# AIM-SE/AC-TSR

Hardware: AMD Instinct MI355X
Metric: user-sequences/sec fwd+bwd, AC-SASRec L=50 d=64, 1/2/4/8 MI355X (higher is better)
Workload: dtype f32; 1 GPU; ACSASRec full training step (spatial + adversarial calibrators, BASELINE configs[2]), synthetic 100000-item catalogue, B=512/GPU L=50 d=64 h=2 2 layers inner=256, CE loss, two-pass backward + Adam; global_batch=512, seq_len=50, hidden=64, heads=2, parallelism=dp1, launch=hipGraph replay per step, backward=two walks (reference protocol, trainer.py:672-686)

## Files before the change

### ac_tsr_amd/_lib.py

```python
from __future__ import annotations

import ctypes as C
import os
import subprocess

_HERE = os.path.dirname(os.path.abspath(__file__))
CSRC = os.path.join(_HERE, "csrc")
LIB_PATH = os.environ.get("ACATTN_LIB") or os.path.join(CSRC, "libacattn.so")
HEADER_PATH = os.path.join(os.path.dirname(_HERE), "include", "acattn.h")

ABI_VERSION = 34
MAX_MASKS = 8
NSTAT = 8
MASK_STRUCTURED, MASK_DENSE_LL, MASK_DENSE_L = 0, 1, 2
COMBINE = {"fixed": 0, "gate": 1, "annealing": 2}
RICH = {"none": 0, "fixed": 1, "trainable": 2}
RNG_EXPLICIT, RNG_COUNTER = 0, 1
FWD_AUTO, FWD_STREAM, FWD_STAGED, FWD_GENERAL, FWD_LONG = 0, 1, 2, 3, 4
BWD_AUTO, BWD_STREAM, BWD_ROW, BWD_LONG = 0, 1, 2, 3

_f = C.c_void_p


class Problem(C.Structure):
# ... 106 lines not shown

class EmbedProblem(C.Structure):
    _fields_ = [("rows", C.c_int32), ("L", C.c_int32), ("H", C.c_int32), ("n_table_rows", C.c_int64), ("idx", _f),
                ("table", _f), ("pos", _f), ("gamma", _f), ("beta", _f), ("eps", C.c_float), ("p_drop", C.c_float),
                ("keep", _f), ("seed", C.c_uint64), ("seed_device", _f), ("nonzero_out", _f), ("hot_id_plus1", C.c_int64)]


EMBED_BWD_CHUNKS = 8
PENALTY_WS_FLOATS = 1024
WGRAD_MAX_GROUP = 8
WGRAD_MAX_REDUCE = 32
SUMROWS_MAX_DEFER = 8

SYMBOLS = {
    "acattn_abi_version": (C.c_int, []),
    "acattn_max_sequence_length": (C.c_int, []),
    "acattn_calibrated_attention_bwd_gate_summed": (C.c_int, [C.POINTER(Problem), C.POINTER(BwdIO)]),
    "acattn_calibrated_attention_bwd_pair_supported": (C.c_int, [C.POINTER(Problem), C.POINTER(BwdIO)]),
    "acattn_last_error": (C.c_char_p, []),
    "acattn_fwd_algorithmic_bytes": (C.c_int64, [C.POINTER(Problem)]),
    "acattn_calibrated_attention_fwd": (C.c_int, [C.POINTER(Problem), C.POINTER(FwdOut), C.c_void_p]),
    "acattn_calibrated_attention_bwd": (C.c_int, [C.POINTER(Problem), C.POINTER(BwdIO), C.c_void_p]),
    "acattn_calibrated_attention_bwd_attack_side": (C.c_int, [C.POINTER(Problem), C.POINTER(BwdIO), C.c_void_p]),
    "acattn_spatial_attention_bwd": (C.c_int, [C.POINTER(Problem), C.POINTER(SpatialBwdIO), C.c_void_p]),
    "acattn_spatial_attention_bwd_workspace_bytes": (C.c_int64, [C.POINTER(Problem)]),
    "acattn_spatial_affines": (C.c_int, [C.POINTER(Problem), _f, C.c_void_p]),
    "acattn_full_sort_ce_workspace_bytes": (C.c_int64, [C.POINTER(CeProblem)]),
    "acattn_full_sort_ce_fwd": (C.c_int, [C.POINTER(CeProblem), _f, _f, _f, C.c_void_p]),
    "acattn_full_sort_ce_fwd_dir": (C.c_int, [C.POINTER(CeProblem), _f, _f, _f, _f, C.c_void_p]),
    "acattn_full_sort_ce_bwd": (C.c_int, [C.POINTER(CeProblem), _f, _f, _f, _f, _f, C.c_void_p]),
    "acattn_full_sort_ce_fwd_pair_workspace_bytes": (C.c_int64, [C.POINTER(CeProblem), C.POINTER(CeProblem)]),
    "acattn_full_sort_ce_fwd_pair": (C.c_int, [C.POINTER(CeProblem), C.POINTER(CeProblem), _f, _f, _f, _f, _f, _f, C.c_void_p]),
    "acattn_full_sort_ce_products": (C.c_int, [C.c_int]),
    "acattn_linear_products": (C.c_int, [C.c_int]),
    "acattn_dropout_add_layernorm_fwd": (C.c_int, [C.POINTER(LnProblem), _f, _f, C.c_void_p]),
    "acattn_dropout_add_layernorm_bwd": (C.c_int, [C.POINTER(LnProblem), _f, _f, _f, _f, _f, C.c_void_p]),
    "acattn_embed_layernorm_fwd": (C.c_int, [C.POINTER(EmbedProblem), _f, _f, C.c_void_p]),
    "acattn_embed_layernorm_bwd": (C.c_int, [C.POINTER(EmbedProblem), _f, _f, C.c_int64, _f, _f, _f, C.c_void_p]),
    "acattn_projections_supported": (C.c_int, [C.c_int32, C.c_int32]),
    "acattn_projections_bwd_workspace_bytes": (C.c_int64, [C.POINTER(ProjProblem)]),
    "acattn_projections_fwd": (C.c_int, [C.POINTER(ProjProblem), C.POINTER(ProjOut), C.c_void_p]),
    "acattn_projections_qkv_supported": (C.c_int, [C.c_int32]),
    "acattn_projections_qkv_fwd": (C.c_int, [C.POINTER(ProjProblem), C.POINTER(ProjOut), C.c_void_p]),
    "acattn_projections_bwd": (C.c_int, [C.POINTER(ProjProblem), C.POINTER(ProjBwdIO), C.c_void_p]),
    "acattn_layer_tail_supported": (C.c_int, [C.c_int32, C.c_int32]),
    "acattn_layer_tail_fwd": (C.c_int, [C.POINTER(TailProblem), C.POINTER(TailSaved), C.c_void_p]),
# ... 99 lines not shown
```

### ac_tsr_amd/csrc/acattn_api.hip

```cpp
#include <stdint.h>
#include <stdio.h>
#include <string.h>

#include <algorithm>

#include "acattn_common.h"

namespace {
thread_local char g_err[256] = "";
constexpr int ACATTN_MAX_L = 496;

int fail(const char* msg) {
  snprintf(g_err, sizeof(g_err), "%s", msg);
  return -1;
}

int check_problem(const acattn_problem* p) {
  if (!p) return fail("problem is NULL");
  if (p->B < 1 || p->L < 1 || p->H < 1 || p->n_heads < 1) return fail("B, L, H, n_heads must be positive");
  if (p->H % p->n_heads != 0)
    return fail("The hidden size is not a multiple of the number of attention heads");
  const int dh = p->H / p->n_heads;
  if (dh != 16 && dh != 32 && dh != 64 && dh != 128) return fail("unsupported head size: dh must be 16, 32, 64 or 128");
  if (p->L > ACATTN_MAX_L) return fail("unsupported sequence length: L must be <= 496 (acattn_max_sequence_length)");
// ... 15 lines not shown
    if (p->adversarial && !p->two_level && !p->keep_before) return fail("explicit dropout needs keep_before");
  }
  if (p->adversarial) {
    if (!p->qa || !p->ka) return fail("adversarial calibrator needs qa and ka");
    if (p->rng_mode == ACATTN_RNG_EXPLICIT && !p->noise) return fail("explicit rng mode needs noise");
    if (p->combine_option == ACATTN_COMBINE_GATE) {
      if (!p->gate_logits) return fail("combine_option gate needs gate_logits");
    } else if (p->combine_option != ACATTN_COMBINE_FIXED && p->combine_option != ACATTN_COMBINE_ANNEALING) {
      return fail("unknown combine_option");
    }
    if (!p->two_level) {
      if (p->rich_combine != ACATTN_RICH_FIXED && p->rich_combine != ACATTN_RICH_TRAINABLE)
        return fail("unknown rich_calibrated_combine");
      if (p->rich_combine == ACATTN_RICH_TRAINABLE && !p->rich_ratio) return fail("trainable rich combine needs rich_ratio");
    }
  }
  return 0;
}
}

void acattn_set_error(const char* msg) { snprintf(g_err, sizeof(g_err), "%s", msg); }

int acattn_launch_bwd_attack(const acattn_problem& p, const acattn_bwd_io& io, hipStream_t stream, float* gate_zero);

extern "C" {

int acattn_abi_version(void) { return ACATTN_ABI_VERSION; }

int acattn_max_sequence_length(void) { return ACATTN_MAX_L; }

int acattn_select_forward_kernel(int which) { return acattn_fwd_kernel_choice(which); }

int acattn_select_backward_kernel(int which) { return acattn_bwd_kernel_choice(which); }

const char* acattn_last_error(void) { return g_err; }

int64_t acattn_fwd_algorithmic_bytes(const acattn_problem* p) {
  if (!p) return -1;
  const int64_t t_lh = 4LL * p->L * p->H, t_ll = 4LL * p->L * p->L;
  if (!p->adversarial) return (int64_t)p->B * 4 * t_lh;
  int64_t per_seq = 7 * t_lh + (int64_t)p->n_heads * t_ll;
  if (p->combine_option == ACATTN_COMBINE_GATE) per_seq += t_ll;
  return (int64_t)p->B * per_seq;
}

int acattn_calibrated_attention_fwd(const acattn_problem* p, const acattn_fwd_out* out, void* stream) {
// ... 24 lines not shown
int acattn_calibrated_attention_bwd(const acattn_problem* p, const acattn_bwd_io* io, void* stream) {
  if (int rc = check_problem(p)) return rc;
  if (!io) return fail("io is NULL");
  if (!p->adversarial) return fail("backward is defined for the adversarial (full) operator only");
  if (!io->attack_mask || !io->row_stats) return fail("backward needs the forward's attack_mask and row_stats");
  if (!io->dq || !io->dk || !io->dv || !io->dqa || !io->dka) return fail("dq, dk, dv, dqa, dka must be non-NULL");
  if (p->combine_option == ACATTN_COMBINE_GATE && !io->dgate_logits) return fail("gate combine needs dgate_logits");
  if (!io->dw_order_part || !io->dw_dist_part || !io->dsmall_part) return fail("parameter partial buffers must be non-NULL");
  if (io->part_stride != 0 && io->part_stride < 2 * (p->H / p->n_heads)) return fail("part_stride is smaller than a partial row");
  const int rc = acattn_launch_bwd(*p, *io, (hipStream_t)stream);
  if (rc > 0) snprintf(g_err, sizeof(g_err), "HIP launch failed: %s", hipGetErrorString((hipError_t)rc));
  return rc;
}

int acattn_calibrated_attention_bwd_attack_side(const acattn_problem* p, const acattn_bwd_io* io, void* stream) {
  if (int rc = check_problem(p)) return rc;
  if (!io) return fail("io is NULL");
  if (!p->adversarial) return fail("backward is defined for the adversarial (full) operator only");
  if (!io->attack_mask || !io->row_stats) return fail("backward needs the forward's attack_mask and row_stats");
  if (!io->dqa || !io->dka) return fail("dqa, dka must be non-NULL");
  const int rc = acattn_launch_bwd_attack(*p, *io, (hipStream_t)stream, nullptr);
  if (rc > 0) snprintf(g_err, sizeof(g_err), "HIP launch failed: %s", hipGetErrorString((hipError_t)rc));
  if (rc == -100) snprintf(g_err, sizeof(g_err), "the attack-side backward (acattn_bwd_attack.hip) does not cover this launch");
  return rc;
}

int acattn_calibrated_attention_bwd_gate_summed(const acattn_problem* p, const acattn_bwd_io* io) {
  if (!p || !io || p->B < 1 || p->L < 1 || p->H < 1 || p->n_heads < 1) return 0;
  return acattn_bwd_gate_summed(*p, *io) ? 1 : 0;
}

int acattn_calibrated_attention_bwd_pair_supported(const acattn_problem* p, const acattn_bwd_io* io) {
  if (!p || !io || p->B < 1 || p->L < 1 || p->H < 1 || p->n_heads < 1) return 0;
  return acattn_bwd_pair_supported(*p, *io) ? 1 : 0;
}

int64_t acattn_calibrated_attention_bwd_workspace_bytes(const acattn_problem* p) {
  if (!p || p->B < 1 || p->L < 1 || p->n_heads < 1) return -1;
  const bool long_form = p->L > 208 || acattn_bwd_kernel_choice(-1) == ACATTN_BWD_LONG;
  return (long_form ? 2 : 1) * acattn_bwd_stream_ws_bytes(*p);
}

int acattn_spatial_attention_bwd(const acattn_problem* p, const acattn_spatial_bwd_io* io, void* stream) {
  if (int rc = check_problem(p)) return rc;
  if (!io) return fail("io is NULL");
  if (p->L > 208) return fail("the spatial-only backward is built for sequence length L <= 208 (the long form covers the forward and acattn_calibrated_attention_bwd)");
// ... 592 lines not shown
```

### ac_tsr_amd/csrc/acattn_bwd.hip

```cpp
#include <stdlib.h>

#include "acattn_common.h"

int acattn_launch_bwd_general_dh16(const acattn_problem& p, const acattn_bwd_io& io, hipStream_t stream);
int acattn_launch_bwd_general_dh32(const acattn_problem& p, const acattn_bwd_io& io, hipStream_t stream);
int acattn_launch_bwd_general_dh64(const acattn_problem& p, const acattn_bwd_io& io, hipStream_t stream);
int acattn_launch_bwd_general_dh128(const acattn_problem& p, const acattn_bwd_io& io, hipStream_t stream);

int acattn_launch_bwd_fast(const acattn_problem& p, const acattn_bwd_io& io, hipStream_t stream);
int acattn_launch_bwd_stream(const acattn_problem& p, const acattn_bwd_io& io, hipStream_t stream);
int acattn_launch_bwd_attack(const acattn_problem& p, const acattn_bwd_io& io, hipStream_t stream, float* gate_zero = nullptr);
int acattn_launch_bwd_onerow(const acattn_problem& p, const acattn_bwd_io& io, bool accumulate, hipStream_t stream, bool gate_zeroed = false);
int acattn_launch_bwd_long(const acattn_problem& p, const acattn_bwd_io& io, hipStream_t stream);

namespace {
thread_local int g_bwd_kernel = ACATTN_BWD_AUTO;
}
int acattn_bwd_kernel_choice(int which) {
  const int old = g_bwd_kernel;
  if (which >= ACATTN_BWD_AUTO && which <= ACATTN_BWD_LONG) g_bwd_kernel = which;
  return old;
}

bool acattn_bwd_onerow_applies(const acattn_problem& p, const acattn_bwd_io& io);

namespace {
bool attack_kernel_enabled() {
  static const bool on = getenv("ACATTN_BWD_ATTACK") ? atoi(getenv("ACATTN_BWD_ATTACK")) != 0 : true;
  return on;
}
bool onerow_split_applies(const acattn_problem& p, const acattn_bwd_io& io) {
  static const bool split = getenv("ACATTN_ONEROW_SPLIT") ? atoi(getenv("ACATTN_ONEROW_SPLIT")) != 0 : true;
  if (!(split && (io.d_attack_mask || io.d_penalty_part) && io.read_rows && io.n_read_rows == 1 && !io.active_qblocks && !io.attack_only && p.L <= 64))
    return false;
// ... 51 lines not shown
      if (rc_mask == 0) {
        acattn_bwd_io row_io = io;
        row_io.d_attack_mask = nullptr;
        row_io.d_penalty_part = nullptr;
        const int rc_row = acattn_launch_bwd_onerow(p, row_io, true, stream, gate_zeroed);
        if (rc_row != -100) return rc_row;
        acattn_set_error("attention backward: the mask-only launch ran but the one-row kernel does not cover this problem (read-row chain not computed)");
        return -1;
      }
      if (rc_mask != -100) return rc_mask;
    }
    if (io.dgate_summed) {
      acattn_set_error("attention backward: dgate_summed was accepted but no one-row form ran");
      return -1;
    }
  }
  static const bool short_stream = getenv("ACATTN_BWD_SHORT_STREAM") && atoi(getenv("ACATTN_BWD_SHORT_STREAM")) != 0;
  const bool short_rows = p.L <= 64 && !short_stream;
  if (which == ACATTN_BWD_AUTO && short_rows) {
    if (io.attack_only && attack_kernel_enabled()) {
      const int rc_attack = acattn_launch_bwd_attack(p, io, stream);
      if (rc_attack != -100) return rc_attack;
    }
    const int rc_fast = acattn_launch_bwd_fast(p, io, stream);
    if (rc_fast != -100) return rc_fast;
  }
  if (which == ACATTN_BWD_AUTO || which == ACATTN_BWD_STREAM) {
    const int rc_stream = acattn_launch_bwd_stream(p, io, stream);
    if (rc_stream != -100) return rc_stream;
  }
  const int rc_fast = acattn_launch_bwd_fast(p, io, stream);
  if (rc_fast != -100) return rc_fast;
  switch (p.H / p.n_heads) {
    case 16: return acattn_launch_bwd_general_dh16(p, io, stream);
    case 32: return acattn_launch_bwd_general_dh32(p, io, stream);
    case 64: return acattn_launch_bwd_general_dh64(p, io, stream);
    case 128: return acattn_launch_bwd_general_dh128(p, io, stream);
  }
  return -1;
}
```

### ac_tsr_amd/csrc/acattn_bwd_attack.hip

```cpp
#include <stdlib.h>

#include <type_traits>

#include "acattn_common.h"

namespace {

constexpr float kLog2e = 1.44269504088896340736f;
constexpr float kLn2 = 0.69314718055994530942f;

__device__ __forceinline__ float ex2(float x) { return __builtin_amdgcn_exp2f(x); }
__device__ __forceinline__ float hsum(const f4 v) { return (v[0] + v[1]) + (v[2] + v[3]); }

constexpr int TS = 20;

__device__ __forceinline__ int again(int x) {
  asm volatile("" : "+v"(x));
  return x;
}

__device__ __forceinline__ void rng_keep_pair(const RngKey key, uint32_t row_id, uint32_t grp, float p_drop, uint32_t& keep_after,
                                              uint32_t& keep_mask) {
  if (p_drop == 0.5f) {
    uint32_t x = (row_id * 64u + grp) ^ key.a;
    x *= 0x7feb352dU;
    x ^= x >> 15;
    x *= 0x846ca68bU;
    x ^= x >> 16;
    x += key.b;
    const uint32_t w2 = rng_word(x, 0xB5297A4Du, 0x85EBCA77u);
    keep_after = (w2 >> 4) & 0xFu;
    keep_mask = (w2 >> 12) & 0xFu;
  } else {
    const RngGroup rg = rng_group(key, row_id, grp, p_drop);
    keep_after = rg.keep_after;
    keep_mask = rg.keep_mask;
  }
}

template <int DH, bool CTX>
__global__ void __launch_bounds__(256, CTX ? 3 : 4) acattn_bwd_attack_kernel(const acattn_problem P, const acattn_bwd_io IO, float* gate_zero,
                                                                    const int n_slots) {
  constexpr int KS = DH / 4;
  constexpr int DT = DH / 16;
  constexpr int VS = DH + 4;
  constexpr int SLOT = 16 * VS;

  const int L = P.L, H = P.H, nh = P.n_heads;
  const int nT = (L + 15) >> 4;
  const int LP = nT * 16;
  int b, h;
  decode_block(blockIdx.x, P.B, nh, b, h);
  const int lane = threadIdx.x & 63;
  const int wave = __builtin_amdgcn_readfirstlane(threadIdx.x >> 6);
  const int c = lane & 15, g = lane >> 4;
  const size_t rowbase = (size_t)b * L;
  const int hoff = h * DH;
  const size_t bh = (size_t)b * nh + h;

  extern __shared__ __attribute__((aligned(16))) float smem[];
// ... 486 lines not shown
```

### ac_tsr_amd/csrc/acattn_common.h

```cpp
#pragma once
#include <hip/hip_runtime.h>
#include <stdint.h>

#include <type_traits>

#include "acattn.h"

typedef float f4 __attribute__((ext_vector_type(4)));
typedef float f4u __attribute__((ext_vector_type(4), aligned(4)));

#define ACATTN_NEG_INF (-__builtin_inff())
#define ACATTN_MASK_FILL (-10000.0f)
#define ACATTN_LOG_EPS (1e-24f)

__device__ __forceinline__ float quad_sum(float x) {
  auto r = __builtin_amdgcn_permlane16_swap(__float_as_uint(x), __float_as_uint(x), false, false);
  x = __uint_as_float(r[0]) + __uint_as_float(r[1]);
  auto s = __builtin_amdgcn_permlane32_swap(__float_as_uint(x), __float_as_uint(x), false, false);
  return __uint_as_float(s[0]) + __uint_as_float(s[1]);
}

__device__ __forceinline__ float quad_max(float x) {
  auto r = __builtin_amdgcn_permlane16_swap(__float_as_uint(x), __float_as_uint(x), false, false);
  x = fmaxf(__uint_as_float(r[0]), __uint_as_float(r[1]));
// ... 157 lines not shown
    const float u2 = (float)(wn[pair] & 0xFFFFu) * (1.0f / 65536.0f);
    const float rad = __builtin_amdgcn_sqrtf(__builtin_amdgcn_logf(u1) * (-2.0f * 0.69314718055994530942f)) * scale;
    acattn_f2 cs = {__builtin_amdgcn_cosf(u2), __builtin_amdgcn_sinf(u2)};
    asm("" : "+v"(cs));
    n[pair] = cs * rad;
  }
  o.n01 = n[0];
  o.n23 = n[1];
  const uint32_t w2 = rng_word(x, 0xB5297A4Du, 0x85EBCA77u);
  o.keep_after = (w2 >> 4) & 0xFu;
  o.keep_mask = (w2 >> 12) & 0xFu;
  o.keep_before = (w2 >> 20) & 0xFu;
  return o;
}

__device__ __forceinline__ uint32_t rng_keep_mask_half(const RngKey key, uint32_t row_id, uint32_t grp) {
  uint32_t x = (row_id * 64u + grp) ^ key.a;
  x *= 0x7feb352dU;
  x ^= x >> 15;
  x *= 0x846ca68bU;
  x ^= x >> 16;
  x += key.b;
  return (rng_word(x, 0xB5297A4Du, 0x85EBCA77u) >> 12) & 0xFu;
}

__device__ __forceinline__ f4 keep_scale4(uint32_t bits, float keep_scale) {
  f4 s;
#pragma unroll
  for (int r = 0; r < 4; ++r) s[r] = ((bits >> r) & 1u) ? keep_scale : 0.f;
  return s;
}
__device__ __forceinline__ int sbit(uint32_t bits, int idx) {
  int m = __builtin_amdgcn_sbfe(bits, idx, 1);
  asm("" : "+v"(m));
  return m;
}
__device__ __forceinline__ float keep_and(float x, uint32_t bits, int r) {
  return __uint_as_float(__float_as_uint(x) & (uint32_t)sbit(bits, r));
}

__device__ __forceinline__ void store_out4(float* p, const f4 v) { __builtin_nontemporal_store(v, (f4*)p); }
__device__ __forceinline__ void store_out1(float* p, const float v) { __builtin_nontemporal_store(v, p); }

__device__ __forceinline__ bool qblock_has_ctx(const acattn_bwd_io& IO, int b, int qb) {
  if (IO.active_qblocks) return (IO.active_qblocks[b] >> qb) & 1u;
  if (IO.read_rows) {
// ... 130 lines not shown
```

### include/acattn.h

```cpp
#ifndef ACATTN_H_
#define ACATTN_H_

#include <stdint.h>

#ifdef __cplusplus
extern "C" {
#endif

#define ACATTN_ABI_VERSION 34

enum {
  ACATTN_MASK_STRUCTURED = 0,
  ACATTN_MASK_DENSE_LL = 1,
  ACATTN_MASK_DENSE_L = 2
};

enum { ACATTN_COMBINE_FIXED = 0, ACATTN_COMBINE_GATE = 1, ACATTN_COMBINE_ANNEALING = 2 };

enum { ACATTN_RICH_NONE = 0, ACATTN_RICH_FIXED = 1, ACATTN_RICH_TRAINABLE = 2 };

enum {
  ACATTN_RNG_EXPLICIT = 0,
  ACATTN_RNG_COUNTER = 1
};
// ... 369 lines not shown
                           uint8_t* keep_after, uint8_t* keep_mask, uint8_t* keep_before, void* stream);

enum {
  ACATTN_FWD_AUTO = 0,
  ACATTN_FWD_STREAM = 1,
  ACATTN_FWD_STAGED = 2,
  ACATTN_FWD_GENERAL = 3,
  ACATTN_FWD_LONG = 4
};
int acattn_select_forward_kernel(int which);

int acattn_max_sequence_length(void);

enum {
  ACATTN_BWD_AUTO = 0,
  ACATTN_BWD_STREAM = 1,
  ACATTN_BWD_ROW = 2,
  ACATTN_BWD_LONG = 3
};
int acattn_select_backward_kernel(int which);

int acattn_calibrated_attention_bwd_attack_side(const acattn_problem* p, const acattn_bwd_io* io, void* stream);

#ifdef __cplusplus
}
#endif
#endif
```

Measured before the change: 540,500 user-sequences/sec.

## Add specialised calibrated-walk attention backward kernel for short sequences

Adds a new fused backward kernel for the calibrated (non-attack) walk of the two-pass backward. It is dispatched ahead of the generic fast backward when L<=64, the mask is structured, gate combine and two-level are set, and RNG is counter-based. The kernel keeps K, Ka and V in LDS, computes the spatial and score gradients per 16-row query block with MFMA, and reduces the key-side gradients through LDS slots, either all at once or in turns when LDS is short. The aim is to replace the general kernel with one that avoids redundant traffic and launches for this shape, at the cost of a large new code path and high LDS use that may limit occupancy.

Result: no change. 545,600 user-sequences/sec, median of 6 (+0.9%).

```diff
diff --git a/ac_tsr_amd/_lib.py b/ac_tsr_amd/_lib.py
--- a/ac_tsr_amd/_lib.py
+++ b/ac_tsr_amd/_lib.py
@@ -152,6 +152,7 @@
     "acattn_calibrated_attention_fwd": (C.c_int, [C.POINTER(Problem), C.POINTER(FwdOut), C.c_void_p]),
     "acattn_calibrated_attention_bwd": (C.c_int, [C.POINTER(Problem), C.POINTER(BwdIO), C.c_void_p]),
     "acattn_calibrated_attention_bwd_attack_side": (C.c_int, [C.POINTER(Problem), C.POINTER(BwdIO), C.c_void_p]),
+    "acattn_calibrated_attention_bwd_cal": (C.c_int, [C.POINTER(Problem), C.POINTER(BwdIO), C.c_void_p]),
     "acattn_spatial_attention_bwd": (C.c_int, [C.POINTER(Problem), C.POINTER(SpatialBwdIO), C.c_void_p]),
     "acattn_spatial_attention_bwd_workspace_bytes": (C.c_int64, [C.POINTER(Problem)]),
     "acattn_spatial_affines": (C.c_int, [C.POINTER(Problem), _f, C.c_void_p]),
diff --git a/ac_tsr_amd/csrc/acattn_api.hip b/ac_tsr_amd/csrc/acattn_api.hip
--- a/ac_tsr_amd/csrc/acattn_api.hip
+++ b/ac_tsr_amd/csrc/acattn_api.hip
@@ -61,6 +61,7 @@
 void acattn_set_error(const char* msg) { snprintf(g_err, sizeof(g_err), "%s", msg); }
 
 int acattn_launch_bwd_attack(const acattn_problem& p, const acattn_bwd_io& io, hipStream_t stream, float* gate_zero);
+int acattn_launch_bwd_cal(const acattn_problem& p, const acattn_bwd_io& io, hipStream_t stream);
 
 extern "C" {
 
@@ -131,6 +132,19 @@
   const int rc = acattn_launch_bwd_attack(*p, *io, (hipStream_t)stream, nullptr);
   if (rc > 0) snprintf(g_err, sizeof(g_err), "HIP launch failed: %s", hipGetErrorString((hipError_t)rc));
   if (rc == -100) snprintf(g_err, sizeof(g_err), "the attack-side backward (acattn_bwd_attack.hip) does not cover this launch");
+  return rc;
+}
+
+int acattn_calibrated_attention_bwd_cal(const acattn_problem* p, const acattn_bwd_io* io, void* stream) {
+  if (int rc = check_problem(p)) return rc;
+  if (!io) return fail("io is NULL");
+  if (!p->adversarial) return fail("backward is defined for the adversarial (full) operator only");
+  if (!io->attack_mask || !io->row_stats) return fail("backward needs the forward's attack_mask and row_stats");
+  if (!io->dq || !io->dk || !io->dv || !io->dqa || !io->dka) return fail("dq, dk, dv, dqa, dka must be non-NULL");
+  if (io->part_stride != 0 && io->part_stride < 2 * (p->H / p->n_heads)) return fail("part_stride is smaller than a partial row");
+  const int rc = acattn_launch_bwd_cal(*p, *io, (hipStream_t)stream);
+  if (rc > 0) snprintf(g_err, sizeof(g_err), "HIP launch failed: %s", hipGetErrorString((hipError_t)rc));
+  if (rc == -100) snprintf(g_err, sizeof(g_err), "the calibrated-walk backward (acattn_bwd_cal.hip) does not cover this launch");
   return rc;
 }
 
diff --git a/ac_tsr_amd/csrc/acattn_bwd.hip b/ac_tsr_amd/csrc/acattn_bwd.hip
--- a/ac_tsr_amd/csrc/acattn_bwd.hip
+++ b/ac_tsr_amd/csrc/acattn_bwd.hip
@@ -10,6 +10,7 @@
 int acattn_launch_bwd_fast(const acattn_problem& p, const acattn_bwd_io& io, hipStream_t stream);
 int acattn_launch_bwd_stream(const acattn_problem& p, const acattn_bwd_io& io, hipStream_t stream);
 int acattn_launch_bwd_attack(const acattn_problem& p, const acattn_bwd_io& io, hipStream_t stream, float* gate_zero = nullptr);
+int acattn_launch_bwd_cal(const acattn_problem& p, const acattn_bwd_io& io, hipStream_t stream);
 int acattn_launch_bwd_onerow(const acattn_problem& p, const acattn_bwd_io& io, bool accumulate, hipStream_t stream, bool gate_zeroed = false);
 int acattn_launch_bwd_long(const acattn_problem& p, const acattn_bwd_io& io, hipStream_t stream);
 
@@ -107,6 +108,10 @@
       const int rc_attack = acattn_launch_bwd_attack(p, io, stream);
       if (rc_attack != -100) return rc_attack;
     }
+    if (!io.attack_only) {
+      const int rc_cal = acattn_launch_bwd_cal(p, io, stream);
+      if (rc_cal != -100) return rc_cal;
+    }
     const int rc_fast = acattn_launch_bwd_fast(p, io, stream);
     if (rc_fast != -100) return rc_fast;
   }
diff --git a/ac_tsr_amd/csrc/acattn_bwd_attack.hip b/ac_tsr_amd/csrc/acattn_bwd_attack.hip
--- a/ac_tsr_amd/csrc/acattn_bwd_attack.hip
+++ b/ac_tsr_amd/csrc/acattn_bwd_attack.hip
@@ -17,25 +17,6 @@
 __device__ __forceinline__ int again(int x) {
   asm volatile("" : "+v"(x));
   return x;
-}
-
-__device__ __forceinline__ void rng_keep_pair(const RngKey key, uint32_t row_id, uint32_t grp, float p_drop, uint32_t& keep_after,
-                                              uint32_t& keep_mask) {
-  if (p_drop == 0.5f) {
-    uint32_t x = (row_id * 64u + grp) ^ key.a;
-    x *= 0x7feb352dU;
-    x ^= x >> 15;
-    x *= 0x846ca68bU;
-    x ^= x >> 16;
-    x += key.b;
-    const uint32_t w2 = rng_word(x, 0xB5297A4Du, 0x85EBCA77u);
-    keep_after = (w2 >> 4) & 0xFu;
-    keep_mask = (w2 >> 12) & 0xFu;
-  } else {
-    const RngGroup rg = rng_group(key, row_id, grp, p_drop);
-    keep_after = rg.keep_after;
-    keep_mask = rg.keep_mask;
-  }
 }
 
 template <int DH, bool CTX>
diff --git a/ac_tsr_amd/csrc/acattn_bwd_cal.hip b/ac_tsr_amd/csrc/acattn_bwd_cal.hip
--- /dev/null
+++ b/ac_tsr_amd/csrc/acattn_bwd_cal.hip
@@ -0,0 +1,686 @@
+#include <stdlib.h>
+
+#include <type_traits>
+
+#include "acattn_common.h"
+
+namespace {
+
+constexpr float kLog2e = 1.44269504088896340736f;
+
+__device__ __forceinline__ float ex2(float x) { return __builtin_amdgcn_exp2f(x); }
+__device__ __forceinline__ float hsum(const f4 v) { return (v[0] + v[1]) + (v[2] + v[3]); }
+
+__device__ __forceinline__ float row16_sum(float v) {
+  v += __builtin_bit_cast(float, __builtin_amdgcn_update_dpp(0, __builtin_bit_cast(int, v), 0xB1, 0xF, 0xF, false));
+  v += __builtin_bit_cast(float, __builtin_amdgcn_update_dpp(0, __builtin_bit_cast(int, v), 0x4E, 0xF, 0xF, false));
+  v += __builtin_bit_cast(float, __builtin_amdgcn_update_dpp(0, __builtin_bit_cast(int, v), 0x141, 0xF, 0xF, false));
+  v += __builtin_bit_cast(float, __builtin_amdgcn_update_dpp(0, __builtin_bit_cast(int, v), 0x140, 0xF, 0xF, false));
+  return v;
+}
+
+__device__ __forceinline__ uint32_t again(uint32_t x) {
+  asm volatile("" : "+v"(x));
+  return x;
+}
+
+constexpr int TS = 20;
+
+#ifdef ACATTN_BWD_STAMPS
+__device__ unsigned long long g_bwd_cal_stamps[8192 * 16];
+#define BWD_STAMP(k)                                                                  \
+  do {                                                                                \
+    __builtin_amdgcn_sched_barrier(0);                                                \
+    asm volatile("s_memtime %0\n\ts_waitcnt lgkmcnt(0)" : "=s"(stamp_[k])::"memory"); \
+    __builtin_amdgcn_sched_barrier(0);                                                \
+  } while (0)
+#else
+#define BWD_STAMP(k)
+#endif
+
+template <int DH>
+__global__ void __launch_bounds__(256, 2) acattn_bwd_cal_kernel(const acattn_problem P, const acattn_bwd_io IO, const int n_slots) {
+  constexpr int KS = DH / 4;
+  constexpr int DT = DH / 16;
+  constexpr int VS = DH + 4;
+  constexpr int SLOT = 16 * VS;
+  constexpr int CP = 2 * DH + 4;
+
+  const int L = P.L, H = P.H, nh = P.n_heads;
+  const int nT = (L + 15) >> 4;
+  const int LP = nT * 16;
+  int b, h;
+  decode_block(blockIdx.x, P.B, nh, b, h);
+  const int lane = threadIdx.x & 63;
+  const int wave = __builtin_amdgcn_readfirstlane(threadIdx.x >> 6);
+  const int c = lane & 15, g = lane >> 4;
+  const size_t rowbase = (size_t)b * L;
+  const int hoff = h * DH;
+  const size_t bh = (size_t)b * nh + h;
+#ifdef ACATTN_BWD_STAMPS
+  unsigned long long stamp_[16] = {};
+#endif
+  BWD_STAMP(0);
+
+  extern __shared__ __attribute__((aligned(16))) float smem[];
+  float* Ks = smem;
+  float* Kas = Ks + LP * VS;
+  float* Vs = Kas + LP * VS;
+  float* slots_k = smem;
+  float* slots_ka = slots_k + n_slots * SLOT;
+  float* slots_v = smem + max(3 * LP * VS, 2 * n_slots * SLOT);
+  float* s_co = slots_v + n_slots * SLOT;
+  float* s_cd = s_co + LP;
+  float* s_km = s_cd + LP;
+  float* s_lt = s_km + LP;
+  float* s_kh = s_lt + LP;
+  float* scr_all = s_kh + nT * 2 * DH;
+  float* part_all = scr_all + nT * 16 * TS;
+  float* scr = scr_all + wave * 16 * TS;
+  float* my_part = part_all + wave * (2 * LP + CP);
+  const int PW = 2 * LP + CP;
+
+  const int qb = wave;
+  const int i0 = qb * 16, i = i0 + c;
+  const bool row_ok = i < L;
+  float qf[KS], qaf[KS];
+  {
+    const size_t off = (rowbase + (row_ok ? i : 0)) * H + hoff + KS * g;
+#pragma unroll
+    for (int s4 = 0; s4 < KS / 4; ++s4) {
+      f4 t = {0.f, 0.f, 0.f, 0.f}, ta = t;
+      if (row_ok) {
+        t = *(const f4*)(P.q + off + 4 * s4);
+        ta = *(const f4*)(P.qa + off + 4 * s4);
+      }
+#pragma unroll
+      for (int e = 0; e < 4; ++e) {
+        qf[4 * s4 + e] = t[e];
+        qaf[4 * s4 + e] = ta[e];
+      }
+    }
+  }
+  float lse_x2 = 0.f, lse_y2 = 0.f, lse_v2 = 0.f, lse_w2 = 0.f;
+  if (row_ok) {
+    const float* sp = IO.row_stats + (bh * L + i) * ACATTN_NSTAT;
+    lse_x2 = sp[0] * kLog2e;
+    lse_y2 = sp[1] * kLog2e;
+    lse_v2 = sp[3] * kLog2e;
+    lse_w2 = sp[4] * kLog2e;
+  }
+
+  constexpr int KV_IT = DH / 16;
+  f4 r_k[KV_IT], r_ka[KV_IT], r_v[KV_IT];
+#pragma unroll
+  for (int it = 0; it < KV_IT; ++it) {
+    const int idx = threadIdx.x + it * blockDim.x;
+    const int row = idx / (DH / 4), c4 = idx - row * (DH / 4);
+    r_k[it] = f4{0.f, 0.f, 0.f, 0.f};
+    r_ka[it] = r_k[it];
+    r_v[it] = r_k[it];
+    if (row < L) {
+      const size_t o = (rowbase + row) * H + hoff + 4 * c4;
+      r_k[it] = *(const f4*)(P.k + o);
+      r_ka[it] = *(const f4*)(P.ka + o);
+      r_v[it] = *(const f4*)(P.v + o);
+    }
+  }
+  const f4 w_ko = *(const f4*)(P.w_order + DH + 4 * (threadIdx.x % (DH / 4)));
+  const f4 w_kd = *(const f4*)(P.w_dist + DH + 4 * (threadIdx.x % (DH / 4)));
+  const uint8_t r_valid = (threadIdx.x < L) ? P.key_valid[rowbase + threadIdx.x] : (uint8_t)0;
+  BWD_STAMP(1);
+#pragma unroll
+  for (int it = 0; it < KV_IT; ++it) {
+    const int idx = threadIdx.x + it * blockDim.x;
+    const int row = idx / (DH / 4), c4 = idx - row * (DH / 4);
+    const f4 kv = r_k[it];
+    *(f4*)(Ks + row * VS + 4 * c4) = kv;
+    *(f4*)(Kas + row * VS + 4 * c4) = r_ka[it];
+    *(f4*)(Vs + row * VS + 4 * c4) = r_v[it];
+    float co = kv.x * w_ko.x + kv.y * w_ko.y + kv.z * w_ko.z + kv.w * w_ko.w;
+    float cd = kv.x * w_kd.x + kv.y * w_kd.y + kv.z * w_kd.z + kv.w * w_kd.w;
+#pragma unroll
+    for (int off = 1; off < DH / 4; off <<= 1) {
+      co += __shfl_xor(co, off);
+      cd += __shfl_xor(cd, off);
+    }
+    if (c4 == 0) {
+      s_co[row] = -kLog2e * co;
+      s_cd[row] = cd;
+    }
+  }
+  if (threadIdx.x < LP) {
+    const int j = threadIdx.x;
+    float km = ACATTN_NEG_INF;
+    if (j < L) km = r_valid ? 0.f : ACATTN_MASK_FILL * kLog2e;
+    s_km[j] = km;
+    s_lt[j] = logf((float)(j + 1));
+  }
+
+  float ao = 0.f, ad = 0.f;
+#pragma unroll
+  for (int s4 = 0; s4 < KS / 4; ++s4) {
+    const f4 a = *(const f4*)(P.w_order + KS * g + 4 * s4), d = *(const f4*)(P.w_dist + KS * g + 4 * s4);
+#pragma unroll
+    for (int e = 0; e < 4; ++e) {
+      ao += qf[4 * s4 + e] * a[e];
+      ad += qf[4 * s4 + e] * d[e];
+    }
+  }
+  ao = quad_sum(ao) + P.b_order[0];
+  ad = quad_sum(ad) + P.b_dist[0];
+  const float sc = P.scalar[0];
+  const uint64_t seed_eff = P.seed + (P.seed_device ? *P.seed_device : 0ull);
+  const RngKey rkey = rng_key(seed_eff);
+  __syncthreads();
+  BWD_STAMP(2);
+
+  const unsigned long long valid_keys = __ballot(lane < L && s_km[lane] == 0.f);
+  const int first_valid = valid_keys ? __ffsll((long long)valid_keys) - 1 : L;
+  const bool causal = P.causal != 0;
+  const int nt_valid = valid_keys ? ((63 - __clzll((long long)valid_keys)) >> 4) + 1 : nT;
+  auto tiles_of_block = [&](int q) {
+    const bool rows_see_a_key = causal ? first_valid <= 16 * q : valid_keys != 0;
+    return rows_see_a_key ? min(causal ? min(nT, q + 1) : nT, nt_valid) : nT;
+  };
+  int nts[4], base[4], total = 0;
+#pragma unroll
+  for (int q = 0; q < 4; ++q) {
+    nts[q] = q < nT ? tiles_of_block(q) : 0;
+    base[q] = total;
+    total += nts[q];
+  }
+  const int nt = tiles_of_block(qb);
+  const int my_base = qb == 0 ? base[0] : qb == 1 ? base[1] : qb == 2 ? base[2] : base[3];
+  const bool in_turns = total > n_slots;
+
+  const float s2 = sc * sc;
+  const float inv_sqrt = 1.0f / sqrtf((float)DH);
+  const float scale2 = inv_sqrt * kLog2e;
+  const float ao2 = -kLog2e * ao;
+  const float nc2 = -(0.5f * s2 * scale2);
+  const bool has_drop = P.p_drop > 0.f;
+  const float keep_scale = has_drop ? 1.0f / (1.0f - P.p_drop) : 1.0f;
+  const uint32_t prow = ((uint32_t)bh * L + (row_ok ? i : 0)) * (uint32_t)L;
+  const uint32_t rng_row = (uint32_t)(bh * L + i);
+  const float okf = row_ok ? 1.0f : 0.0f;
+
+  auto mask4 = [&](int t) -> f4 {
+    const f4 km4 = *(const f4*)(s_km + 16 * t + 4 * g);
+    if (causal && (16 * t + 15 > i0)) {
+      const int dq = (c - 4 * g) + 16 * (qb - t);
+      f4 m;
+#pragma unroll
+      for (int r = 0; r < 4; ++r) m[r] = (dq < r) ? fminf(km4[r], ACATTN_MASK_FILL * kLog2e) : km4[r];
+      return m;
+    }
+    return km4;
+  };
+  auto spatial = [&](int t, f4& pr, f4& val, f4& df) {
+    const f4 ea = *(const f4*)(s_co + 16 * t + 4 * g) + ao2;
+    const f4 cd4 = *(const f4*)(s_cd + 16 * t + 4 * g);
+    const int d0 = i - (16 * t + 4 * g);
+    f4 lt4;
+    if (16 * t + 15 > i0) {
+#pragma unroll
+      for (int r = 0; r < 4; ++r) {
+        pr[r] = fast_rcp(1.0f + ex2(ea[r]));
+        val[r] = (d0 - r < 0) ? pr[r] : 1.0f - pr[r];
+        lt4[r] = s_lt[d0 - r < 0 ? r - d0 : d0 - r];
+      }
+    } else {
+      const float* lp = s_lt + d0;
+#pragma unroll
+      for (int r = 0; r < 4; ++r) {
+        pr[r] = fast_rcp(1.0f + ex2(ea[r]));
+        val[r] = 1.0f - pr[r];
+        lt4[r] = lp[-r];
+      }
+    }
+    df = lt4 - (cd4 + ad);
+  };
+  auto load_seg = [&](const float* base, int t) -> f4 {
+    const int j0 = 16 * t + 4 * g;
+    f4 v = {0.f, 0.f, 0.f, 0.f};
+    if (row_ok && j0 < L) {
+      const float* p = base + j0;
+      if (j0 + 3 < L) {
+        v = *(const f4u*)p;
+      } else {
+#pragma unroll
+        for (int r = 0; r < 4; ++r)
+          if (j0 + r < L) v[r] = p[r];
+      }
+    }
+    return v;
+  };
+  auto store_seg = [&](float* base, int t, const f4 val) {
+    const int j0 = 16 * t + 4 * g;
+    if (!row_ok || j0 >= L) return;
+    float* p = base + j0;
+    if (j0 + 3 < L) {
+      *(f4u*)p = val;
+    } else {
+#pragma unroll
+      for (int r = 0; r < 4; ++r)
+        if (j0 + r < L) p[r] = val[r];
+    }
+  };
+  auto load_cols = [&](const float* src, float (&col)[4][DT]) {
+#pragma unroll
+    for (int s = 0; s < 4; ++s) {
+      const int row = i0 + 4 * g + s;
+      const float* p = src + (rowbase + min(row, L - 1)) * H + hoff + c;
+#pragma unroll
+      for (int dt = 0; dt < DT; ++dt) col[s][dt] = row < L ? p[16 * dt] : 0.f;
+    }
+  };
+
+  auto body = [&](auto ntb_c) {
+    constexpr int NTB = decltype(ntb_c)::value;
+    asm volatile("; %0 key tiles" ::"n"(NTB) : "memory");
+
+    auto score_tiles = [&](const float* Xs, const float (&frag)[KS], f4 (&out)[NTB]) {
+#pragma unroll
+      for (int t = 0; t < NTB; ++t) out[t] = f4{0.f, 0.f, 0.f, 0.f};
+#pragma unroll
+      for (int s4 = 0; s4 < KS / 4; ++s4) {
+#pragma unroll
+        for (int t = 0; t < NTB; ++t) {
+          const f4 x4 = *(const f4*)(Xs + (16 * t + c) * VS + KS * g + 4 * s4);
+#pragma unroll
+          for (int e = 0; e < 4; ++e) out[t] = mfma16(x4[e], frag[4 * s4 + e], out[t]);
+        }
+      }
+    };
+    auto key_side = [&](const f4 (&tile)[NTB], const float (&col)[4][DT], auto sink) {
+#pragma unroll
+      for (int t = 0; t < NTB; ++t) {
+        asm volatile("s_waitcnt lgkmcnt(0)" ::: "memory");
+        *(f4*)(scr + c * TS + 4 * g) = tile[t];
+        asm volatile("s_waitcnt lgkmcnt(0)" ::: "memory");
+        f4 o[DT];
+#pragma unroll
+        for (int dt = 0; dt < DT; ++dt) o[dt] = f4{0.f, 0.f, 0.f, 0.f};
+#pragma unroll
+        for (int s = 0; s < 4; ++s) {
+          const float b_t = scr[(4 * g + s) * TS + c];
+#pragma unroll
+          for (int dt = 0; dt < DT; ++dt) o[dt] = mfma16(col[s][dt], b_t, o[dt]);
+        }
+        sink(t, o);
+      }
+    };
+    auto park = [&](const f4 (&tile)[NTB], const float (&col)[4][DT], float* area) {
+      if (!in_turns) {
+        key_side(tile, col, [&](int t, const f4 (&o)[DT]) {
+          float* sl = area + (my_base + t) * SLOT + c * VS + 4 * g;
+#pragma unroll
+          for (int dt = 0; dt < DT; ++dt) *(f4*)(sl + 16 * dt) = o[dt];
+        });
+      } else {
+        for (int j = lane; j < SLOT; j += 64) area[wave * SLOT + j] = 0.f;
+        __syncthreads();
+        for (int q = 0; q < nT; ++q) {
+          if (q == qb)
+            key_side(tile, col, [&](int t, const f4 (&o)[DT]) {
+              float* sl = area + t * SLOT + c * VS + 4 * g;
+#pragma unroll
+              for (int dt = 0; dt < DT; ++dt) *(f4*)(sl + 16 * dt) += o[dt];
+            });
+          __syncthreads();
+        }
+      }
+    };
+
+    constexpr bool EARLY = DH <= 32;
+    f4 gc[KS / 4];
+    float gcc[4][DT];
+    auto load_gc = [&] {
+      const size_t off = (rowbase + (row_ok ? i : 0)) * H + hoff + KS * g;
+#pragma unroll
+      for (int s4 = 0; s4 < KS / 4; ++s4) {
+        gc[s4] = f4{0.f, 0.f, 0.f, 0.f};
+        if (row_ok) gc[s4] = *(const f4*)(IO.d_ctx_calibrated + off + 4 * s4);
+      }
+    };
+    if constexpr (EARLY) {
+      load_gc();
+      load_cols(IO.d_ctx_calibrated, gcc);
+    }
+
+    f4 tS[NTB], tM[NTB];
+    score_tiles(Ks, qf, tS);
+    score_tiles(Kas, qaf, tM);
+#pragma unroll
+    for (int t = 0; t < NTB; ++t) {
+      const f4 mk4 = mask4(t);
+      f4 pr, val, df;
+      spatial(t, pr, val, df);
+      f4 lg;
+#pragma unroll
+      for (int r = 0; r < 4; ++r) lg[r] = __builtin_amdgcn_logf(val[r] + ACATTN_LOG_EPS);
+      f4 x = tS[t] * scale2 + mk4;
+      x = lg * inv_sqrt + x;
+      x = (df * df) * nc2 + x;
+#pragma unroll
+      for (int r = 0; r < 4; ++r) tS[t][r] = ex2(x[r] - lse_x2) * okf;
+      const f4 y = tM[t] * scale2 + mk4;
+#pragma unroll
+      for (int r = 0; r < 4; ++r) tM[t][r] = ex2(y[r] - lse_y2) * okf;
+    }
+    BWD_STAMP(3);
+
+    uint32_t keepA = 0, keepM = 0;
+#pragma unroll
+    for (int t = 0; t < NTB; ++t) {
+      uint32_t ka = 0xFu, km = 0xFu;
+      if (has_drop) rng_keep_pair(rkey, rng_row, (uint32_t)(4 * t + g), P.p_drop, ka, km);
+      keepA |= ka << (4 * t);
+      keepM |= km << (4 * t);
+    }
+    BWD_STAMP(4);
+
+    f4 dPa[NTB], dMa[NTB];
+    {
+      f4 dAw[NTB], Ac[NTB], Aw[NTB];
+#pragma unroll
+      for (int t = 0; t < NTB; ++t) dAw[t] = f4{0.f, 0.f, 0.f, 0.f};
+      if constexpr (!EARLY) load_gc();
+#pragma unroll
+      for (int s4 = 0; s4 < KS / 4; ++s4) {
+#pragma unroll
+        for (int t = 0; t < NTB; ++t) {
+          const f4 x4 = *(const f4*)(Vs + (16 * t + c) * VS + KS * g + 4 * s4);
+#pragma unroll
+          for (int e = 0; e < 4; ++e) dAw[t] = mfma16(x4[e], gc[s4][e], dAw[t]);
+        }
+      }
+      const float* grow = P.gate_logits + (rowbase + (row_ok ? i : 0)) * L;
+      float dc = 0.f;
+#pragma unroll
+      for (int t = 0; t < NTB; ++t) {
+        const f4 sa = keep_scale4((keepA >> (4 * t)) & 0xFu, keep_scale), sm = keep_scale4((keepM >> (4 * t)) & 0xFu, keep_scale);
+        const f4 p = tS[t] * sa, m = tM[t] * sm;
+        const f4 mk4 = mask4(t);
+        const f4 a1 = m * (-kLog2e) + kLog2e;
+        f4 ex1;
+#pragma unroll
+        for (int r = 0; r < 4; ++r) ex1[r] = ex2(a1[r]);
+        const f4 v2 = (p * ex1) * kLog2e + (mk4 - lse_v2);
+        const f4 gt = gate_value(load_seg(grow, t), P.gate_is_prob);
+#pragma unroll
+        for (int r = 0; r < 4; ++r) Ac[t][r] = ex2(v2[r]) * okf;
+        const f4 w2 = (gt * (p - Ac[t]) + Ac[t]) * kLog2e + (mk4 - lse_w2);
+#pragma unroll
+        for (int r = 0; r < 4; ++r) Aw[t][r] = ex2(w2[r]) * okf;
+        dc += hsum(Aw[t] * dAw[t]);
+      }
+      dc = quad_sum(dc);
+      if constexpr (!EARLY) load_cols(IO.d_ctx_calibrated, gcc);
+      park(Aw, gcc, slots_v);
+      float r1 = 0.f;
+      keepA = again(keepA);
+#pragma unroll
+      for (int t = 0; t < NTB; ++t) {
+        const f4 sa = keep_scale4((keepA >> (4 * t)) & 0xFu, keep_scale);
+        const f4 p = tS[t] * sa;
+        const f4 gt = gate_value(load_seg(grow, t), P.gate_is_prob);
+        const f4 dw = Aw[t] * (dAw[t] - dc);
+        store_seg(IO.dgate_logits + prow, t, dw * (p - Ac[t]) * (gt * (1.0f - gt)));
+        dPa[t] = gt * dw;
+        const f4 dac = (1.0f - gt) * dw;
+        dAw[t] = dac;
+        r1 += hsum(Ac[t] * dac);
+      }
+      for (int t = NTB; t < nT; ++t) store_seg(IO.dgate_logits + prow, t, f4{0.f, 0.f, 0.f, 0.f});
+      r1 = quad_sum(r1);
+      keepA = again(keepA);
+      keepM = again(keepM);
+#pragma unroll
+      for (int t = 0; t < NTB; ++t) {
+        const f4 sa = keep_scale4((keepA >> (4 * t)) & 0xFu, keep_scale), sm = keep_scale4((keepM >> (4 * t)) & 0xFu, keep_scale);
+        const f4 p = tS[t] * sa, m = tM[t] * sm;
+        const f4 a1 = m * (-kLog2e) + kLog2e;
+        f4 ex1;
+#pragma unroll
+        for (int r = 0; r < 4; ++r) ex1[r] = ex2(a1[r]);
+        const f4 dv = Ac[t] * (dAw[t] - r1);
+        dPa[t] += dv * ex1;
+        dMa[t] = -(dv * (p * ex1));
+      }
+    }
+    BWD_STAMP(5);
+
+    float r2 = 0.f, r3 = 0.f;
+    keepA = again(keepA);
+    keepM = again(keepM);
+#pragma unroll
+    for (int t = 0; t < NTB; ++t) {
+      dMa[t] *= keep_scale4((keepM >> (4 * t)) & 0xFu, keep_scale);
+      r2 += hsum(tM[t] * dMa[t]);
+      dPa[t] *= keep_scale4((keepA >> (4 * t)) & 0xFu, keep_scale);
+      r3 += hsum(tS[t] * dPa[t]);
+    }
+    r2 = quad_sum(r2);
+    r3 = quad_sum(r3);
+    float da_o = 0.f, da_d = 0.f, dsc = 0.f;
+#pragma unroll
+    for (int t = 0; t < NTB; ++t) {
+      dMa[t] = (tM[t] * (dMa[t] - r2)) * inv_sqrt;
+      dPa[t] = (tS[t] * (dPa[t] - r3)) * inv_sqrt;
+      f4 pr, val, df;
+      spatial(t, pr, val, df);
+      f4 d_o, d_d;
+#pragma unroll
+      for (int r = 0; r < 4; ++r) {
+        const float sgn = (16 * t + 4 * g + r > i) ? 1.0f : -1.0f;
+        d_o[r] = dPa[t][r] * (sgn * pr[r] * (1.0f - pr[r])) * fast_rcp(val[r] + ACATTN_LOG_EPS);
+      }
+      d_d = dPa[t] * (df * s2);
+      dsc += hsum(dPa[t] * (df * df)) * (-sc);
+      da_o += hsum(d_o);
+      da_d += hsum(d_d);
+#pragma unroll
+      for (int r = 0; r < 4; ++r) {
+        d_o[r] = row16_sum(d_o[r]);
+        d_d[r] = row16_sum(d_d[r]);
+      }
+      if (c == 0) {
+        *(f4*)(my_part + 16 * t + 4 * g) = d_o;
+        *(f4*)(my_part + LP + 16 * t + 4 * g) = d_d;
+      }
+    }
+    da_o = quad_sum(da_o);
+    da_d = quad_sum(da_d);
+    dsc = quad_sum(dsc);
+#pragma unroll
+    for (int s = 0; s < KS; ++s) {
+      const float vo = row16_sum(da_o * qf[s]), vd = row16_sum(da_d * qf[s]);
+      if (c == 0) {
+        my_part[2 * LP + KS * g + s] = vo;
+        my_part[2 * LP + DH + KS * g + s] = vd;
+      }
+    }
+    {
+      const float so = row16_sum(da_o), sd = row16_sum(da_d), ss = row16_sum(dsc);
+      if (lane == 0) *(f4*)(my_part + 2 * LP + 2 * DH) = f4{so, sd, ss, 0.f};
+    }
+    BWD_STAMP(6);
+
+    float qc[4][DT], qac[4][DT];
+    load_cols(P.q, qc);
+    load_cols(P.qa, qac);
+    {
+      f4 oq[DT], oqa[DT];
+#pragma unroll
+      for (int dt = 0; dt < DT; ++dt) {
+        oq[dt] = f4{0.f, 0.f, 0.f, 0.f};
+        oqa[dt] = oq[dt];
+      }
+#pragma unroll
+      for (int t = 0; t < NTB; ++t)
+#pragma unroll
+        for (int r = 0; r < 4; ++r) {
+          const float* kp = Ks + (16 * t + 4 * g + r) * VS + c;
+          const float* kap = Kas + (16 * t + 4 * g + r) * VS + c;
+#pragma unroll
+          for (int dt = 0; dt < DT; ++dt) {
+            oq[dt] = mfma16(kp[16 * dt], dPa[t][r], oq[dt]);
+            oqa[dt] = mfma16(kap[16 * dt], dMa[t][r], oqa[dt]);
+          }
+        }
+      if (row_ok) {
+        const uint32_t off = ((uint32_t)rowbase + i) * H + hoff + 4 * g;
+#pragma unroll
+        for (int dt = 0; dt < DT; ++dt) {
+          const f4 wo_lo = *(const f4*)(P.w_order + 16 * dt + 4 * g), wd_lo = *(const f4*)(P.w_dist + 16 * dt + 4 * g);
+          *(f4*)(IO.dq + off + 16 * dt) = oq[dt] + da_o * wo_lo + da_d * wd_lo;
+          *(f4*)(IO.dqa + off + 16 * dt) = oqa[dt];
+        }
+      }
+    }
+    BWD_STAMP(7);
+    __syncthreads();
+    park(dPa, qc, slots_k);
+    park(dMa, qac, slots_ka);
+    BWD_STAMP(8);
+  };
+  switch (nt) {
+    case 1: body(std::integral_constant<int, 1>{}); break;
+    case 2: body(std::integral_constant<int, 2>{}); break;
+    case 3: body(std::integral_constant<int, 3>{}); break;
+    default: body(std::integral_constant<int, 4>{}); break;
+  }
+
+  f4 k_again[KV_IT];
+#pragma unroll
+  for (int it = 0; it < KV_IT; ++it) {
+    const int idx = threadIdx.x + it * blockDim.x;
+    const int row = idx / (DH / 4), c4 = idx - row * (DH / 4);
+    k_again[it] = f4{0.f, 0.f, 0.f, 0.f};
+    if (row < L) k_again[it] = *(const f4*)(P.k + (rowbase + row) * H + hoff + 4 * c4);
+  }
+  const f4 w_ko2 = *(const f4*)(P.w_order + DH + 4 * (int)again(threadIdx.x % (DH / 4)));
+  const f4 w_kd2 = *(const f4*)(P.w_dist + DH + 4 * (int)again(threadIdx.x % (DH / 4)));
+  __syncthreads();
+  BWD_STAMP(9);
+  f4 wo4 = {0.f, 0.f, 0.f, 0.f}, wd4 = wo4;
+#pragma unroll
+  for (int it = 0; it < KV_IT; ++it) {
+    const int idx = threadIdx.x + it * blockDim.x;
+    const int row = idx / (DH / 4), c4 = idx - row * (DH / 4);
+    if (row >= L) continue;
+    const int t = row >> 4, in = (row & 15) * VS + 4 * c4;
+    f4 sk = {0.f, 0.f, 0.f, 0.f}, ska = sk, sv = sk;
+    float so = 0.f, sd = 0.f;
+#pragma unroll
+    for (int q = 0; q < 4; ++q)
+      if (nts[q] > t) {
+        so += part_all[q * PW + row];
+        sd += part_all[q * PW + LP + row];
+        if (!in_turns) {
+          const int o = (base[q] + t) * SLOT + in;
+          sk += *(const f4*)(slots_k + o);
+          ska += *(const f4*)(slots_ka + o);
+          sv += *(const f4*)(slots_v + o);
+        }
+      }
+    if (in_turns) {
+      sk = *(const f4*)(slots_k + t * SLOT + in);
+      ska = *(const f4*)(slots_ka + t * SLOT + in);
+      sv = *(const f4*)(slots_v + t * SLOT + in);
+    }
+    const size_t o = (rowbase + row) * H + hoff + 4 * c4;
+    *(f4*)(IO.dka + o) = ska;
+    *(f4*)(IO.dk + o) = sk + (so * w_ko2 + sd * w_kd2);
+    *(f4*)(IO.dv + o) = sv;
+    wo4 += so * k_again[it];
+    wd4 += sd * k_again[it];
+  }
+#pragma unroll
+  for (int off = DH / 4; off < 64; off <<= 1)
+#pragma unroll
+    for (int e = 0; e < 4; ++e) {
+      wo4[e] += __shfl_xor(wo4[e], off);
+      wd4[e] += __shfl_xor(wd4[e], off);
+    }
+  if (lane < DH / 4) {
+    *(f4*)(s_kh + wave * 2 * DH + 4 * lane) = wo4;
+    *(f4*)(s_kh + wave * 2 * DH + DH + 4 * lane) = wd4;
+  }
+  __syncthreads();
+  for (int d = threadIdx.x; d < 2 * DH; d += blockDim.x) {
+    float wo = 0.f, wd = 0.f;
+    for (int q = 0; q < nT; ++q) {
+      const float* src = d < DH ? part_all + q * PW + 2 * LP + d : s_kh + q * 2 * DH + (d - DH);
+      wo += src[0];
+      wd += src[DH];
+    }
+    IO.dw_order_part[bh * (IO.part_stride ? IO.part_stride : 2 * DH) + d] = wo;
+    IO.dw_dist_part[bh * (IO.part_stride ? IO.part_stride : 2 * DH) + d] = wd;
+  }
+  if (threadIdx.x < 4) {
+    float s = 0.f;
+    if (threadIdx.x < 3)
+      for (int q = 0; q < nT; ++q) s += part_all[q * PW + 2 * LP + 2 * DH + threadIdx.x];
+    IO.dsmall_part[bh * (IO.part_stride ? IO.part_stride : 4) + threadIdx.x] = s;
+  }
+#ifdef ACATTN_BWD_STAMPS
+  BWD_STAMP(10);
+  if (lane == 0 && blockIdx.x * 4 + wave < 8192) {
+    stamp_[11] = (unsigned long long)qb;
+    for (int k = 0; k < 12; ++k) g_bwd_cal_stamps[(blockIdx.x * 4 + wave) * 16 + k] = stamp_[k];
+  }
+#endif
+}
+
+constexpr size_t kLdsLimit = 160 * 1024;
+
+template <int DH>
+int launch_cal(const acattn_problem& p, const acattn_bwd_io& io, hipStream_t stream) {
+  const int nT = (p.L + 15) / 16, LP = nT * 16, VS = DH + 4, SLOT = 16 * VS;
+  auto bytes = [&](int n_slots) {
+    const int area = 3 * LP * VS > 2 * n_slots * SLOT ? 3 * LP * VS : 2 * n_slots * SLOT;
+    return (size_t)(area + n_slots * SLOT + 4 * LP + nT * 2 * DH + nT * 16 * TS + nT * (2 * LP + 2 * DH + 4)) * sizeof(float);
+  };
+  int n_slots = p.causal ? nT * (nT + 1) / 2 : nT * nT;
+  if (bytes(n_slots) > kLdsLimit) n_slots = nT;
+  const size_t lds = bytes(n_slots);
+  if (lds > kLdsLimit) return -100;
+  auto kern = acattn_bwd_cal_kernel<DH>;
+  if (lds > 64 * 1024) {
+    const hipError_t e = hipFuncSetAttribute((const void*)kern, hipFuncAttributeMaxDynamicSharedMemorySize, (int)lds);
+    if (e != hipSuccess) return (int)e;
+  }
+  hipLaunchKernelGGL(kern, dim3(p.B * p.n_heads), dim3(64 * nT), lds, stream, p, io, n_slots);
+  return (int)hipGetLastError();
+}
+
+}
+
+int acattn_launch_bwd_cal(const acattn_problem& p, const acattn_bwd_io& io, hipStream_t stream) {
+  static const bool on = getenv("ACATTN_BWD_CAL") ? atoi(getenv("ACATTN_BWD_CAL")) != 0 : true;
+  if (!on) return -100;
+  const bool ok = p.L >= 1 && p.L <= 64 && (int64_t)p.B * p.n_heads * p.L * p.L < (1LL << 30) && (int64_t)p.B * p.L * p.H < (1LL << 30) &&
+                  p.mask_mode == ACATTN_MASK_STRUCTURED && p.rng_mode == ACATTN_RNG_COUNTER && p.w_order && p.w_dist &&
+                  p.adversarial && p.combine_option == ACATTN_COMBINE_GATE && p.two_level && !io.attack_only &&
+                  io.d_ctx_calibrated && !io.d_ctx_attacked && !io.d_attack_mask && !io.d_penalty_part &&
+                  !(io.read_rows && io.n_read_rows > 0) && !io.active_qblocks && !io.dgate_summed && !io.dqa2 && !io.dka2 &&
+                  !io.d_ctx_calibrated2 && !io.d_penalty_part2 && p.q && p.k && p.v && p.qa && p.ka && p.key_valid && p.gate_logits &&
+                  p.b_order && p.b_dist && p.scalar && io.dq && io.dk && io.dv && io.dqa && io.dka && io.dgate_logits &&
+                  io.dw_order_part && io.dw_dist_part && io.dsmall_part && io.row_stats;
+  if (!ok) return -100;
+  switch (p.H / p.n_heads) {
+    case 16: return launch_cal<16>(p, io, stream);
+    case 32: return launch_cal<32>(p, io, stream);
+    case 64: return launch_cal<64>(p, io, stream);
+  }
+  return -100;
+}
+
+#ifdef ACATTN_BWD_STAMPS
+extern "C" int acattn_debug_bwd_cal_stamps(unsigned long long* host, int n_words) {
+  return (int)hipMemcpyFromSymbol(host, HIP_SYMBOL(g_bwd_cal_stamps), (size_t)n_words * 8);
+}
+#endif
diff --git a/ac_tsr_amd/csrc/acattn_common.h b/ac_tsr_amd/csrc/acattn_common.h
--- a/ac_tsr_amd/csrc/acattn_common.h
+++ b/ac_tsr_amd/csrc/acattn_common.h
@@ -203,6 +203,25 @@
   x ^= x >> 16;
   x += key.b;
   return (rng_word(x, 0xB5297A4Du, 0x85EBCA77u) >> 12) & 0xFu;
+}
+
+__device__ __forceinline__ void rng_keep_pair(const RngKey key, uint32_t row_id, uint32_t grp, float p_drop, uint32_t& keep_after,
+                                              uint32_t& keep_mask) {
+  if (p_drop == 0.5f) {
+    uint32_t x = (row_id * 64u + grp) ^ key.a;
+    x *= 0x7feb352dU;
+    x ^= x >> 15;
+    x *= 0x846ca68bU;
+    x ^= x >> 16;
+    x += key.b;
+    const uint32_t w2 = rng_word(x, 0xB5297A4Du, 0x85EBCA77u);
+    keep_after = (w2 >> 4) & 0xFu;
+    keep_mask = (w2 >> 12) & 0xFu;
+  } else {
+    const RngGroup rg = rng_group(key, row_id, grp, p_drop);
+    keep_after = rg.keep_after;
+    keep_mask = rg.keep_mask;
+  }
 }
 
 __device__ __forceinline__ f4 keep_scale4(uint32_t bits, float keep_scale) {
diff --git a/include/acattn.h b/include/acattn.h
--- a/include/acattn.h
+++ b/include/acattn.h
@@ -415,6 +415,8 @@
 
 int acattn_calibrated_attention_bwd_attack_side(const acattn_problem* p, const acattn_bwd_io* io, void* stream);
 
+int acattn_calibrated_attention_bwd_cal(const acattn_problem* p, const acattn_bwd_io* io, void* stream);
+
 #ifdef __cplusplus
 }
 #endif
```
